# kennychenfs/KataCoffee

Measured on AMD Instinct MI355X. Metric: self-play training rows/sec + MCTS playouts/sec, 5x5 Coffee b6c96 @600 visits, higher is better.
Workload: dtype fp16

## Files before the change

katacoffee_amd/csrc/nn.hip:

```cpp
#include <hip/hip_runtime.h>
#include <hip/hip_ext.h>

#include <algorithm>
#include <cmath>
#include <cstring>
#include <functional>
#include <mutex>
#include <vector>

#include "detmath.h"
#include "engine.h"
#include "kc_board.h"
#include "lds_dma.h"

namespace kc {

typedef _Float16 h16x8 __attribute__((ext_vector_type(8)));
typedef float f32x4 __attribute__((ext_vector_type(4)));

enum { NN_MODE_F16 = 0, NN_MODE_SPLIT3 = 1, NN_MODE_F8C = 2 };
constexpr int F8C_SHIFT = 11;
constexpr float F8C_MAX = 448.0f;
#ifndef KC_F8C_VGPR
#define KC_F8C_VGPR 96
// ... 27 lines not shown
  const float f = std::frexp(m, &e);
  const int s = e - 9 + (f > 0.875f ? 1 : 0);
  return s < -100 ? -100 : (s > 100 ? 100 : s);
}

template <int X_, int Y_, int C_, int NB_ = NN_BOARDS_PER_WG, int MODE_ = 0, bool BL_ = false>
struct NNGeo {
  static constexpr int X = X_, Y = Y_, C = C_, A = X_ * Y_;
  static constexpr int NB = NB_;
  static constexpr int NW = 8, NT = NW * 64;
  static constexpr int MODE = MODE_;
  static constexpr bool SPLIT = MODE_ != NN_MODE_F16;
  static constexpr int PLANES = SPLIT ? 2 : 1;
  static constexpr bool BL = BL_;
  static constexpr bool F8W = MODE_ == NN_MODE_F8C && KC_F8C_CVTW;
  static constexpr bool F8X = MODE_ == NN_MODE_F8C && KC_F8C_CVTX;
  static constexpr int RING = BL ? ((F8W || F8X) ? 3 : 2) : ((NB_ == NN_SMALL_NB && !SPLIT) ? 4 : 3);
  static constexpr bool PAIRS = RING == 4;
  static constexpr int ROWS = NB * A;
  static constexpr int RT = (ROWS + 15) / 16;
  static constexpr int RGROUPS = NW / 2;
  static constexpr int MAXT = (RT + RGROUPS - 1) / RGROUPS;
  static constexpr int MROWS = RGROUPS * MAXT * 16;
  static constexpr int PX = X + 2, PY = Y + 2, PA = PX * PY;
  static constexpr int ZROW = MROWS;
  static constexpr int PROWS = BL ? MROWS + 1 : NB * PA;
  static constexpr int ASTR = C + 16;
  static constexpr int ROWB = ASTR * 2;
  static constexpr int NCT = C / 32;
  static constexpr int NCT_ALL = C / 16;
  static constexpr int P = 4 * A;
  static constexpr int PLANE_BYTES = (PROWS * ROWB + 15) / 16 * 16;
  static constexpr int ROWB2 = F8X ? ROWB / 2 : ROWB;
  static constexpr int PLANE2_BYTES = SPLIT ? (PROWS * ROWB2 + 15) / 16 * 16 : 0;
  static constexpr int ACT_BYTES = PLANE_BYTES + PLANE2_BYTES;
  static constexpr int SCR = 36;
  static constexpr int OFF_SCR = MROWS * SCR * 4 > 96 * 64 * 4 ? MROWS * SCR * 4 : 96 * 64 * 4;
  static constexpr int OFF_POOL = ACT_BYTES;
  static constexpr int OFF_BIAS = OFF_POOL + 2 * NB * 96 * 4;
  static constexpr int WBUF = (C / 32) * NCT_ALL * 64;
  static constexpr int WBUF2 = !SPLIT ? 0 : (F8W ? WBUF / 2 : WBUF);
  static constexpr int WSLOT = (BL && !SPLIT) ? 3 * WBUF : WBUF + WBUF2;
  static constexpr int SLOT_PIECES = WSLOT / 64;
  static constexpr int tapPieces(int ncb) { return ncb * NCT_ALL * (!SPLIT ? 2 : (F8W ? 3 : 4)) / 2; }
  static constexpr int chunkTaps(int ncb, int ntaps) {
    return SLOT_PIECES / tapPieces(ncb) < 1 ? 1 : (SLOT_PIECES / tapPieces(ncb) < ntaps ? SLOT_PIECES / tapPieces(ncb) : ntaps);
  }
  static constexpr int chunks(int ncb, int ntaps) { return (ntaps + chunkTaps(ncb, ntaps) - 1) / chunkTaps(ncb, ntaps); }
  static constexpr int firstChunkPieces(int ncb, int ntaps) { return chunkTaps(ncb, ntaps) * tapPieces(ncb); }
  static constexpr int NTAB = 2 * MROWS + ROWS;
  static constexpr int OFF_TAB = OFF_BIAS + NB * 64 * 4;
  static constexpr int RING_VH = (32 + 64) * 96 * 4;
  static constexpr int NPRM = NN_PRM;
  static constexpr int OFF_PRM = (OFF_TAB + NTAB * 2 + 15) / 16 * 16;
  static constexpr int OFF_W = OFF_PRM + 2 * NPRM * 4;
  static constexpr int LDS = OFF_W + RING * WSLOT * 16;
  static constexpr bool SCR_IN_RING = BL && !SPLIT;
  static constexpr int SCR_OFF = SCR_IN_RING ? OFF_W + WSLOT * 16 : OFF_SCR;
  static_assert(C % 32 == 0, "C must be a multiple of 32");
  static_assert(SCR_IN_RING ? (MROWS * SCR * 4 <= WSLOT * 16 && RING == 2 && RING_VH + NB * 64 * 4 <= WSLOT * 16)
                            : OFF_SCR + MROWS * SCR * 4 <= ACT_BYTES,
                "f32 branch scratch must fit in act (or in ring slot 1)");
  static_assert(96 * 64 * 4 <= OFF_SCR, "gpool linear weights must fit below scr");
  static_assert(RING * WSLOT * 16 >= RING_VH + NB * 64 * 4, "head linear weights and vh must fit in the ring");
  static_assert((PLANES - 1) * PLANE_BYTES + (BL ? 0 : 2 * PA * ROWB) + 2 * 64 < 65536,
                "A-read offsets must fit the ds_read immediate");
  static_assert(!BL || C == 96, "borderless instances: b6c96");
  static_assert(LDS <= 163840, "LDS budget");
};

#ifdef KC_NN_PROFILE
__device__ unsigned long long g_nnPhase[4][64];
#define NN_PHASE(i)                                  \
  do {                                               \
    if(blockIdx.x < 4 && threadIdx.x == 0) {         \
      g_nnPhase[blockIdx.x][(i)] = clock64();        \
      if((i) == 0 || (i) == 42)                      \
        g_nnPhase[blockIdx.x][(i) == 0 ? 62 : 63] =  \
            __builtin_amdgcn_s_memrealtime();        \
    }                                                \
  } while(0)
#else
#define NN_PHASE(i) \
  do {              \
  } while(0)
#endif

KC_D uint16_t f16bits(float f) { return __builtin_bit_cast(uint16_t, (_Float16)f); }

template <class G>
KC_D int padCell(int b, int p) {
  const int y = p / G::X, x = p - y * G::X;
  return b * G::PA + (y + 1) * G::PX + x + 1;
}

template <class G>
KC_D void aBases(int (&ab)[G::MAXT], const uint16_t* rowPa, int tstart, int lane) {
#pragma unroll
  for(int t = 0; t < G::MAXT; t++) {
    const int r = (tstart + t) * 16 + (lane & 15);
    ab[t] = ((int)rowPa[r] - G::PX - 1) * G::ROWB + 16 * (lane >> 4);
  }
}

template <int NW>
KC_D void stageTapDma(const h16x8* __restrict__ src, uint32_t slotAddr, int ch, int wave, int lane, int rot = 0) {
  for(int c = (wave + NW - rot % NW) % NW; c < ch; c += NW)
    glds16s(src + c * 64, (uint32_t)lane * 16u, slotAddr + c * 1024);
}

template <class G, int NTAPS, int NCB, int PAR = 0, int DBG = 0, bool ENTRY = true>
KC_D void convTiles(const uint16_t* __restrict__ act, const h16x8* __restrict__ w, h16x8* __restrict__ wl,
                    f32x4 (&acc)[G::MAXT][G::NCT], const int (&ab)[G::MAXT], int cg, int lane, int tid,
                    const h16x8* __restrict__ wNext, int chNext, int nextTaps, int g0 = 0) {
  constexpr int CHP = NCB * G::NCT_ALL;
  constexpr int CH = CHP * G::PLANES;
  constexpr int UNITS = CH * 64;
  constexpr int STEPS = NTAPS * NCB;
  const int wave = __builtin_amdgcn_readfirstlane(tid >> 6);
  const uint32_t ring = ldsAddr(wl);
  auto slotOf = [&](int tap) { return G::PAIRS ? (g0 + tap) & 3 : tap % 3; };
  if(ENTRY && !(DBG & 256)) {
    waitVm<0>();
    __syncthreads();
  }
  const char* actB = reinterpret_cast<const char*>(act);
  const h16x8* wlane = wl + (cg * G::NCT) * 64 + lane;
  h16x8 af[2][G::MAXT], bf[2][G::NCT];
  h16x8 afl[G::SPLIT ? 2 : 1][G::MAXT], bfl[G::SPLIT ? 2 : 1][G::NCT];
  auto loadStep = [&](int st, int buf) {
    const int tap = st / NCB, cb = st - tap * NCB;
    const int tb = NTAPS == 9 ? tap : 4;
    const int aoff = ((tb / 3) * G::PX + tb % 3) * G::ROWB + cb * 64;
    const h16x8* wb = wlane + slotOf(tap) * G::WSLOT + cb * G::NCT_ALL * 64;
#pragma unroll
    for(int ct = 0; ct < G::NCT; ct++) {
      bf[buf][ct] = wb[ct * 64];
// ... 248 lines not shown
    }
    if constexpr(F8C) {
      convertStep(st & 1);
      if((st & 1) && !(DBG & 4))
        f8pair();
    }
    if(chunkEnd && chunk + 1 < NCH && (DBG & 2) && !(DBG & 1))
      request(chunk + R);
    constexpr bool LATE = (F8C && KC_F8C_LATE) || (G::MODE == NN_MODE_SPLIT3 && G::BL && KC_ACC_LATE);
    if(!LATE && st + 1 < STEPS && !(DBG & 16)) {
      if(cb == NCB - 1)
        tapAddr(tap + 1);
      loadStep(st + 1, (st + 1) & 1);
    }
    __builtin_amdgcn_sched_barrier(0);
    const int b = st & 1;
#pragma unroll
    for(int t = 0; t < G::MAXT; t++)
#pragma unroll
      for(int ct = 0; ct < G::NCT; ct++)
        acc[t][ct] = __builtin_amdgcn_mfma_f32_16x16x32_f16(bf[b][ct], af[b][t], acc[t][ct], 0, 0, 0);
    if constexpr(G::MODE == NN_MODE_SPLIT3) {
#pragma unroll
      for(int t = 0; t < G::MAXT; t++)
#pragma unroll
        for(int ct = 0; ct < G::NCT; ct++)
          acc[t][ct] = __builtin_amdgcn_mfma_f32_16x16x32_f16(bfl[b][ct], af[b][t], acc[t][ct], 0, 0, 0);
#pragma unroll
      for(int t = 0; t < G::MAXT; t++)
#pragma unroll
        for(int ct = 0; ct < G::NCT; ct++)
          acc[t][ct] = __builtin_amdgcn_mfma_f32_16x16x32_f16(bf[b][ct], afl[b][t], acc[t][ct], 0, 0, 0);
    }
    if(LATE && st + 1 < STEPS) {
      __builtin_amdgcn_sched_barrier(0);
      if(cb == NCB - 1)
        tapAddr(tap + 1);
      loadStep(st + 1, (st + 1) & 1);
    }
    if constexpr(F8C) {
      if(st == STEPS - 1 && !(st & 1) && !(DBG & 4)) {
#pragma unroll
        for(int t = 0; t < G::MAXT; t++)
          aq[t].hi = i32x4{0, 0, 0, 0};
        f8pair();
      }
    }
    __builtin_amdgcn_sched_barrier(0);
  }
}

typedef _Float16 f16x4 __attribute__((ext_vector_type(4)));

template <int NT>
KC_D void stage96(float* __restrict__ dst, const float* __restrict__ src, int rows, int tid) {
  const int n4 = rows * 24;
  for(int q = tid; q < n4; q += NT)
    reinterpret_cast<float4*>(dst)[q] = reinterpret_cast<const float4*>(src)[q];
}

template <class G>
KC_D f32x4* trunkBase(float* trunk, int wave, int lane) {
  return reinterpret_cast<f32x4*>(trunk) + ((size_t)blockIdx.x * G::NW + wave) * (G::MAXT * G::NCT * 64) + lane;
}
template <class G>
constexpr bool regTrunk() {
  return G::MAXT * G::NCT <= 6 && !(G::MODE == NN_MODE_F8C && KC_F8C_PARK);
}
template <class G>
KC_D void storeTrunk(float* trunk, f32x4 (&reg)[G::MAXT][G::NCT], const f32x4 (&a)[G::MAXT][G::NCT], int wave,
                     int lane) {
  if(regTrunk<G>()) {
#pragma unroll
    for(int t = 0; t < G::MAXT; t++)
#pragma unroll
      for(int ct = 0; ct < G::NCT; ct++)
        reg[t][ct] = a[t][ct];
    return;
  }
  f32x4* p = trunkBase<G>(trunk, wave, lane);
#pragma unroll
  for(int t = 0; t < G::MAXT; t++)
#pragma unroll
    for(int ct = 0; ct < G::NCT; ct++)
      p[(t * G::NCT + ct) * 64] = a[t][ct];
}
template <class G>
KC_D void loadTrunk(f32x4 (&a)[G::MAXT][G::NCT], const f32x4 (&reg)[G::MAXT][G::NCT], float* trunk, int wave,
                    int lane) {
  if(regTrunk<G>()) {
#pragma unroll
    for(int t = 0; t < G::MAXT; t++)
#pragma unroll
      for(int ct = 0; ct < G::NCT; ct++)
        a[t][ct] = reg[t][ct];
    return;
  }
  const f32x4* p = trunkBase<G>(trunk, wave, lane);
#pragma unroll
  for(int t = 0; t < G::MAXT; t++)
#pragma unroll
    for(int ct = 0; ct < G::NCT; ct++)
      a[t][ct] = p[(t * G::NCT + ct) * 64];
}

template <class G>
KC_D void zeroAcc(f32x4 (&a)[G::MAXT][G::NCT]) {
#pragma unroll
  for(int t = 0; t < G::MAXT; t++)
#pragma unroll
    for(int ct = 0; ct < G::NCT; ct++)
      a[t][ct] = f32x4{0.0f, 0.0f, 0.0f, 0.0f};
}
// ... 59 lines not shown
                      int nb = 0) {
  float4 sc[G::NCT], bi[G::NCT];
#pragma unroll
  for(int ct = 0; ct < G::NCT; ct++) {
    const int ch = chOf<G>(cg, ct, lane);
    sc[ct] = *reinterpret_cast<const float4*>(s + ch);
    bi[ct] = *reinterpret_cast<const float4*>(bb + ch);
  }
  float m[G::MAXT];
#pragma unroll
  for(int t = 0; t < G::MAXT; t++) {
    m[t] = 0.0f;
    const int row = (tstart + t) * 16 + (lane & 15);
    if(row >= G::ROWS)
      continue;
#pragma unroll
    for(int ct = 0; ct < G::NCT; ct++) {
      const float y0 = fmaxf((float)v[t][ct][0] * sc[ct].x + bi[ct].x, 0.0f);
      const float y1 = fmaxf((float)v[t][ct][1] * sc[ct].y + bi[ct].y, 0.0f);
      const float y2 = fmaxf((float)v[t][ct][2] * sc[ct].z + bi[ct].z, 0.0f);
      const float y3 = fmaxf((float)v[t][ct][3] * sc[ct].w + bi[ct].w, 0.0f);
      storeAct4<G>(act, (int)rowPa[row], chOf<G>(cg, ct, lane), y0, y1, y2, y3);
      if constexpr(G::MODE == NN_MODE_F8C)
        m[t] = fmaxf(m[t], fmaxf(fmaxf(y0, y1), fmaxf(y2, y3)));
    }
  }
  flagHot<G>(hot, base, nb, tstart, lane, m);
}

template <class G>
KC_D void zeroBorders(uint16_t* act, int tid) {
  constexpr int CH = G::ASTR / 8;
  constexpr int NBORD = G::PA - G::A;
  for(int idx = tid; idx < G::NB * NBORD * CH; idx += G::NT) {
    const int q = idx / CH, c = idx - q * CH;
    const int b = q / NBORD, k = q - b * NBORD;
    int cell;
    if(k < G::PX)
      cell = k;
    else if(k < 2 * G::PX)
      cell = (G::PY - 1) * G::PX + (k - G::PX);
    else {
      const int m = k - 2 * G::PX;
      cell = (1 + (m >> 1)) * G::PX + ((m & 1) ? G::PX - 1 : 0);
    }
#pragma unroll
    for(int pl = 0; pl < G::PLANES; pl++)
      reinterpret_cast<uint4*>(act + pl * (G::PLANE_BYTES / 2) + (b * G::PA + cell) * G::ASTR)[c] = uint4{0u, 0u, 0u, 0u};
  }
}

template <class G>
KC_D void poolBoards(const float* scr, const float* vsrc, float* poolP, float* poolV, float sqOff, int tid) {
  for(int idx = tid; idx < G::NB * 64; idx += G::NT) {
    const int pr = idx >> 1, half = idx & 1;
    const int b = pr >> 5, c = pr & 31;
    const int p0 = half ? (G::A + 1) / 2 : 0, p1 = half ? G::A : (G::A + 1) / 2;
    float s = 0.0f, m = 0.0f, sv = 0.0f;
#pragma unroll 4
    for(int p = p0; p < p1; p++) {
      const int o = (b * G::A + p) * G::SCR + c;
      const float v = scr[o];
      s += v;
      m = v > m ? v : m;
      if(vsrc)
        sv += vsrc[o];
    }
    s = s + asF(partner<5>(bitsF(s)));
    m = fmaxf(m, asF(partner<5>(bitsF(m))));
    if(vsrc)
      sv = sv + asF(partner<5>(bitsF(sv)));
    if(half == 0) {
      const float mean = s / (float)G::A;
      poolP[b * 96 + c] = mean;
      poolP[b * 96 + 32 + c] = mean * (sqOff / 10.0f);
      poolP[b * 96 + 64 + c] = m;
      if(vsrc) {
        const float meanv = sv / (float)G::A;
        poolV[b * 96 + c] = meanv;
        poolV[b * 96 + 32 + c] = meanv * (sqOff / 10.0f);
        poolV[b * 96 + 64 + c] = meanv * ((sqOff * sqOff) / 100.0f - 0.1f);
      }
    }
  }
}

template <class G>
KC_D void linear96(const float* wT, int O, const float* in, float* out, int ostr, const float* bias, bool relu,
                   int tid) {
  const int quads = O >> 2;
  auto dot = [&](int q, int ks, int b) {
    float4 s = float4{0.0f, 0.0f, 0.0f, 0.0f};
    const float* xi = in + b * 96 + ks * 24;
    const float* wi = wT + (ks * 24) * O + 4 * q;
#pragma unroll 4
    for(int i = 0; i < 24; i++) {
      const float4 w4 = *reinterpret_cast<const float4*>(wi + i * O);
      const float xv = xi[i];
      s.x += w4.x * xv;
      s.y += w4.y * xv;
      s.z += w4.z * xv;
      s.w += w4.w * xv;
    }
    return s;
  };
  auto emit = [&](const float4& s, int q, int b) {
    float r[4] = {s.x, s.y, s.z, s.w};
#pragma unroll
    for(int j = 0; j < 4; j++) {
      float v = bias ? bias[4 * q + j] + r[j] : r[j];
      out[b * ostr + 4 * q + j] = relu ? fmaxf(v, 0.0f) : v;
    }
  };
  auto add2 = [](float& x, int lvl) {
    int a0, a1;
    if(lvl == 0)
      swapPair<0>(bitsF(x), a0, a1);
    else
      swapPair<1>(bitsF(x), a0, a1);
    x = asF(a0) + asF(a1);
  };
  if(quads == 16 || quads == 8) {
    const int per = 4 * quads;
    for(int idx = tid; idx < G::NB * per; idx += G::NT) {
      const int q = idx & (quads - 1), ks = (idx / quads) & 3, b = idx / per;
      float4 s = dot(q, ks, b);
      if(quads == 16) {
        add2(s.x, 1);
        add2(s.y, 1);
        add2(s.z, 1);
        add2(s.w, 1);
        add2(s.x, 0);
        add2(s.y, 0);
        add2(s.z, 0);
        add2(s.w, 0);
      } else {
        s.x += asF(partner<2>(bitsF(s.x)));
        s.y += asF(partner<2>(bitsF(s.y)));
        s.z += asF(partner<2>(bitsF(s.z)));
        s.w += asF(partner<2>(bitsF(s.w)));
        add2(s.x, 1);
        add2(s.y, 1);
        add2(s.z, 1);
        add2(s.w, 1);
      }
      if(ks == 0)
        emit(s, q, b);
    }
    return;
  }
  for(int idx = tid; idx < G::NB * quads * 4; idx += G::NT) {
    const int ks = idx & 3, q = (idx >> 2) % quads, b = (idx >> 2) / quads;
    float4 s = dot(q, ks, b);
    s.x += asF(partner<5>(bitsF(s.x)));
    s.y += asF(partner<5>(bitsF(s.y)));
    s.z += asF(partner<5>(bitsF(s.z)));
    s.w += asF(partner<5>(bitsF(s.w)));
    s.x += asF(partner<4>(bitsF(s.x)));
    s.y += asF(partner<4>(bitsF(s.y)));
    s.z += asF(partner<4>(bitsF(s.z)));
    s.w += asF(partner<4>(bitsF(s.w)));
    if(ks == 0)
      emit(s, q, b);
  }
}

KC_D float loadParam(const NNLayout* __restrict__ L, const float* __restrict__ WF, int k, int tid) {
  return tid < NN_PRM ? WF[L->prmSlabs + k * NN_PRM + tid] : 0.0f;
}
static int paramSlabSource(const NNLayout& L, int k, int tid) {
  const int f = tid < 384 ? tid / 96 : (tid < 416 ? 4 : 5), i = tid < 384 ? tid - 96 * f : (tid - 384) & 31;
  if(k < L.nblocks) {
    if(f == 0) return L.bn1s[k] + i;
    if(f == 1) return L.bn1b[k] + i;
    if(f == 2) return L.bn2s[k] + i;
    if(f == 3) return L.bn2b[k] + i;
    if(tid < NN_PRM && L.kinds[k] == 1) return (f == 4 ? L.bngs[k] : L.bngb[k]) + i;
    return -1;
  }
  if(tid >= 288) return -1;
  if(tid < 96) return L.tips + tid;
  if(tid < 192) return L.tipb + tid - 96;
  if(tid < 224) return L.pBiasG + tid - 192;
  if(tid < 256) return L.vBias1 + tid - 224;
  return L.pBias2 + tid - 256;
}

#ifndef KC_NN_KERNEL
#define KC_NN_KERNEL kNNForward
#define KC_NN_KERNEL_ATTR
#endif
template <int X, int Y, int C, int NB, int MODE, bool BL>
__global__ void __launch_bounds__(512, 2) KC_NN_KERNEL_ATTR
    KC_NN_KERNEL(const NNLayout* __restrict__ L, const h16x8* __restrict__ WB, const float* __restrict__ WF,
               const uint16_t* __restrict__ tabs, int n, const int* __restrict__ countDev,
               const int* __restrict__ rowIdx, int inWords, float winLen, const uint64_t* __restrict__ in,
               float* __restrict__ out, float* __restrict__ trunk, int* __restrict__ hot) {
  using G = NNGeo<X, Y, C, NB, MODE, BL>;
  extern __shared__ __attribute__((aligned(16))) char smem[];
  NN_PHASE(0);
  const int count = countDev ? min(*countDev, n) : n;
  const int base = blockIdx.x * G::NB;
  if(base >= count)
    return;
  const int nb = min(G::NB, count - base);
  uint32_t hotMask = ~0u;
  if(G::MODE == NN_MODE_SPLIT3 && hot) {
    hotMask = 0;
    for(int b = 0; b < nb; b++)
      hotMask |= __hip_atomic_load(hot + base + b, __ATOMIC_RELAXED, __HIP_MEMORY_SCOPE_AGENT) ? 1u << b : 0u;
    if(!hotMask)
      return;
  }
  const int tid = threadIdx.x, wave = tid >> 6, lane = tid & 63;
  const int rg = wave >> 1, cg = wave & 1;
  const int tstart = rg * G::MAXT;
  uint16_t* act = reinterpret_cast<uint16_t*>(smem);
  float* actF = reinterpret_cast<float*>(smem);
  float* scr = reinterpret_cast<float*>(smem + G::SCR_OFF);
  float* poolP = reinterpret_cast<float*>(smem + G::OFF_POOL);
  float* poolV = poolP + G::NB * 96;
  float* biasS = reinterpret_cast<float*>(smem + G::OFF_BIAS);
  float* vh = reinterpret_cast<float*>(smem + G::OFF_W + G::RING_VH);
  uint16_t* rowPa = reinterpret_cast<uint16_t*>(smem + G::OFF_TAB);
  uint16_t* rowBP = rowPa + G::MROWS;
  float* prm = reinterpret_cast<float*>(smem + G::OFF_PRM);
  h16x8* wl = reinterpret_cast<h16x8*>(smem + G::OFF_W);
  const float sqOff = sqrtf((float)G::A) - 14.0f;

  {
    constexpr int CH0 = G::tapPieces(1);
    const uint32_t ring = ldsAddr(wl);
    if constexpr(G::BL) {
      constexpr int SC = G::firstChunkPieces(1, 9);
#pragma unroll
      for(int j = 0; j + 1 < G::RING && j < G::chunks(1, 9); j++)
        stageChunk<G::NW>(WB + L->wInit + (size_t)j * SC * 64, ring + j * G::WSLOT * 16, SC, wave, lane);
    } else {
#pragma unroll
      for(int tap = 0; tap < 2; tap++)
        stageTapDma<G::NW>(WB + L->wInit + (size_t)tap * CH0 * 64, ring + tap * G::WSLOT * 16, CH0, wave, lane);
    }
  }
  constexpr int NPK = (G::NPRM + G::NT - 1) / G::NT;
  float pre[NPK];
#pragma unroll
  for(int j = 0; j < NPK; j++)
    pre[j] = loadParam(L, WF, 0, tid + j * G::NT);
  for(int i = tid; i < G::NTAB; i += G::NT)
    rowPa[i] = tabs[i];
  for(int idx = tid; idx < G::ACT_BYTES / 16; idx += G::NT)
    reinterpret_cast<uint4*>(smem)[idx] = uint4{0u, 0u, 0u, 0u};
  __syncthreads();
  {
    static_assert(G::NB <= G::NW, "one wave per board");
    constexpr int NBITS = G::A * NUM_SPATIAL, NWD = (NBITS + 63) / 64;
    const int b = __builtin_amdgcn_readfirstlane(wave);
    if(b < nb) {
      const int src = rowIdx ? rowIdx[base + b] : base + b;
      uint64_t words[NWD];
#pragma unroll
      for(int k = 0; k < NWD; k++)
        words[k] = in[(size_t)src * inWords + k];
#pragma unroll
      for(int k = 0; k < NWD; k++) {
        const int i = k * 64 + lane;
        if(i < NBITS && ((words[k] >> lane) & 1ULL)) {
          const int c = i / G::A, p = i - c * G::A;
          const int row = G::BL ? b * G::A + p : padCell<G>(b, p);
          act[row * G::ASTR + c] = (uint16_t)0x3c00;
          if constexpr(G::MODE == NN_MODE_F8C && !G::F8X)
            reinterpret_cast<uint8_t*>(act)[G::PLANE_BYTES + row * G::ROWB + (c >> 3) * 16 + (c & 7)] = 0x38;
        }
      }
    }
  }
  waitVm<0>();
  __syncthreads();

  NN_PHASE(1);
  int ab[G::MAXT];
  int rb[G::MAXT];
  uint32_t vm[G::MAXT];
  if constexpr(G::BL)
    aRowsBL<G>(rb, vm, tstart, lane);
  else
    aBases<G>(ab, rowPa, tstart, lane);
  f32x4 acc[G::MAXT][G::NCT];
  f32x4 park[G::MAXT][G::NCT];
  zeroAcc<G>(acc);
  if constexpr(G::BL)
    convTilesB<G, 9, 1, 0>(act, WB + L->wInit, wl, acc, rb, vm, cg, lane, tid,
                           L->nblocks > 0 ? WB + L->wConv1[0] : WB + L->wHead,
                           L->nblocks > 0 ? G::firstChunkPieces(G::C / 32, 9) : G::firstChunkPieces(G::C / 32, 1),
                           L->nblocks > 0 ? G::chunks(G::C / 32, 9) : 1, L->sInit);
  else
    convTiles<G, 9, 1, 0, 0, false>(act, WB + L->wInit, wl, acc, ab, cg, lane, tid,
                                    L->nblocks > 0 ? WB + L->wConv1[0] : WB + L->wHead, 3 * G::NCT_ALL * G::PLANES,
                                    L->nblocks > 0 ? 9 : 1, 0);
  {
#pragma unroll
    for(int ct = 0; ct < G::NCT; ct++) {
      const float4 g4 = *reinterpret_cast<const float4*>(WF + L->globInit + chOf<G>(cg, ct, lane));
#pragma unroll
      for(int t = 0; t < G::MAXT; t++) {
        acc[t][ct][0] += g4.x * winLen;
        acc[t][ct][1] += g4.y * winLen;
        acc[t][ct][2] += g4.z * winLen;
        acc[t][ct][3] += g4.w * winLen;
      }
    }
  }
// ... 13 lines not shown
    barrierKeepDma();
    NN_PHASE(3 + 4 * blk);
    const float* P = prm + (blk & 1) * G::NPRM;
    storeBnRelu<G>(act, rowPa, acc, P, P + 96, tstart, cg, lane, hot, base, nb);
    waitVm<0>();
    __syncthreads();
    zeroAcc<G>(acc);
#pragma unroll
    for(int j = 0; j < NPK; j++)
      pre[j] = loadParam(L, WF, blk + 1, tid + j * G::NT);
    NN_PHASE(4 + 4 * blk);
    if constexpr(G::BL)
      convTilesB<G, 9, G::C / 32, G::RING == 2 ? 1 : 0>(act, WB + L->wConv1[blk], wl, acc, rb, vm, cg, lane, tid,
                                                       WB + L->wConv2[blk],
                                                       L->kinds[blk] == 0 ? G::firstChunkPieces(3, 9)
                                                                          : G::firstChunkPieces(2, 9),
                                                       L->kinds[blk] == 0 ? G::chunks(3, 9) : G::chunks(2, 9),
                                                       L->sConv1[blk]);
    else
      convTiles<G, 9, G::C / 32, 1, 0, false>(act, WB + L->wConv1[blk], wl, acc, ab, cg, lane, tid,
                                              WB + L->wConv2[blk],
                                              (L->kinds[blk] == 0 ? 3 : 2) * G::NCT_ALL * G::PLANES, 9, 9 + 18 * blk);
#pragma unroll
    for(int j = 0; j < NPK; j++)
      if(tid + j * G::NT < G::NPRM)
        prm[((blk + 1) & 1) * G::NPRM + tid + j * G::NT] = pre[j];
    __syncthreads();
    NN_PHASE(5 + 4 * blk);
    const bool lastBlk = blk + 1 == L->nblocks;
    const h16x8* nextW = lastBlk ? WB + L->wHead : WB + L->wConv1[lastBlk ? 0 : blk + 1];
    const int nextTaps = lastBlk ? 1 : 9;
    if(L->kinds[blk] == 0) {
      f32x4 tr[G::MAXT][G::NCT];
      loadTrunk<G>(tr, park, trunk, wave, lane);
      storeBnRelu<G>(act, rowPa, acc, P + 192, P + 288, tstart, cg, lane, hot, base, nb);
#pragma unroll
      for(int t = 0; t < G::MAXT; t++)
#pragma unroll
        for(int ct = 0; ct < G::NCT; ct++)
          acc[t][ct] = tr[t][ct];
      waitVm<0>();
      __syncthreads();
      NN_PHASE(6 + 4 * blk);
      if constexpr(G::BL)
        convTilesB<G, 9, G::C / 32, 0>(act, WB + L->wConv2[blk], wl, acc, rb, vm, cg, lane, tid, nextW,
                                       G::firstChunkPieces(G::C / 32, nextTaps), G::chunks(G::C / 32, nextTaps),
                                       L->sConv2[blk]);
      else
        convTiles<G, 9, G::C / 32, 0, 0, false>(act, WB + L->wConv2[blk], wl, acc, ab, cg, lane, tid, nextW,
                                                3 * G::NCT_ALL * G::PLANES, nextTaps, 18 + 18 * blk);
      if(!lastBlk)
        storeTrunk<G>(trunk, park, acc, wave, lane);
    } else {
      const float* gs = P + 384;
      const float* gbias = P + 416;
      constexpr int LW = (96 * 64 / 4 + G::NT - 1) / G::NT;
      float4 lw[LW];
      {
        const float4* src = reinterpret_cast<const float4*>(WF + L->linG[blk]);
#pragma unroll
        for(int k = 0; k < LW; k++) {
          const int q = tid + k * G::NT;
          lw[k] = q < Cr * 24 ? src[q] : float4{0.0f, 0.0f, 0.0f, 0.0f};
        }
      }
#pragma unroll
      for(int ct = 0; ct < G::NCT; ct++) {
        const int ch = chOf<G>(cg, ct, lane);
        if(cg * (G::C / 2) + ct * 16 < Cr)
          continue;
        const int gc = ch - Cr;
        const float4 sc = *reinterpret_cast<const float4*>(gs + gc);
        const float4 bi = *reinterpret_cast<const float4*>(gbias + gc);
#pragma unroll
        for(int t = 0; t < G::MAXT; t++) {
          const int row = (tstart + t) * 16 + (lane & 15);
          if(row >= G::ROWS)
            continue;
          *reinterpret_cast<float4*>(scr + (int)rowBP[row] * G::SCR + gc) =
              float4{fmaxf(acc[t][ct][0] * sc.x + bi.x, 0.0f), fmaxf(acc[t][ct][1] * sc.y + bi.y, 0.0f),
                     fmaxf(acc[t][ct][2] * sc.z + bi.z, 0.0f), fmaxf(acc[t][ct][3] * sc.w + bi.w, 0.0f)};
        }
      }
      __syncthreads();
      NN_PHASE(50);
      float* lgT = actF;
#pragma unroll
      for(int k = 0; k < LW; k++) {
        const int q = tid + k * G::NT;
        if(q < Cr * 24)
          reinterpret_cast<float4*>(lgT)[q] = lw[k];
      }
      poolBoards<G>(scr, nullptr, poolP, poolV, sqOff, tid);
      __syncthreads();
      NN_PHASE(51);
      linear96<G>(lgT, Cr, poolP, biasS, Cr, nullptr, false, tid);
      __syncthreads();
      f32x4 tr[G::MAXT][G::NCT];
      loadTrunk<G>(tr, park, trunk, wave, lane);
      if constexpr(G::BL)
        zeroRowBL<G>(act, tid);
      else
        zeroBorders<G>(act, tid);
      NN_PHASE(52);
      {
        const float* s2 = P + 192;
        const float* b2 = P + 288;
        float m[G::MAXT] = {};
#pragma unroll
        for(int ct = 0; ct < G::NCT; ct++) {
          if(cg * (G::C / 2) + ct * 16 >= Cr)
            continue;
          const int ch = chOf<G>(cg, ct, lane);
          const float4 sc = *reinterpret_cast<const float4*>(s2 + ch);
          const float4 bi = *reinterpret_cast<const float4*>(b2 + ch);
#pragma unroll
          for(int t = 0; t < G::MAXT; t++) {
            const int row = (tstart + t) * 16 + (lane & 15);
            if(row >= G::ROWS)
              continue;
            const float4 gb = *reinterpret_cast<const float4*>(biasS + ((int)rowBP[row] / G::A) * Cr + ch);
            const float y0 = fmaxf((acc[t][ct][0] + gb.x) * sc.x + bi.x, 0.0f);
            const float y1 = fmaxf((acc[t][ct][1] + gb.y) * sc.y + bi.y, 0.0f);
            const float y2 = fmaxf((acc[t][ct][2] + gb.z) * sc.z + bi.z, 0.0f);
            const float y3 = fmaxf((acc[t][ct][3] + gb.w) * sc.w + bi.w, 0.0f);
            storeAct4<G>(act, (int)rowPa[row], ch, y0, y1, y2, y3);
            if constexpr(G::MODE == NN_MODE_F8C)
              m[t] = fmaxf(m[t], fmaxf(fmaxf(y0, y1), fmaxf(y2, y3)));
          }
        }
        flagHot<G>(hot, base, nb, tstart, lane, m);
      }
#pragma unroll
      for(int t = 0; t < G::MAXT; t++)
#pragma unroll
        for(int ct = 0; ct < G::NCT; ct++)
          acc[t][ct] = tr[t][ct];
      waitVm<0>();
      __syncthreads();
      NN_PHASE(6 + 4 * blk);
      if constexpr(G::BL)
        convTilesB<G, 9, (G::C - 32) / 32, 0>(act, WB + L->wConv2[blk], wl, acc, rb, vm, cg, lane, tid, nextW,
                                              G::firstChunkPieces(G::C / 32, nextTaps),
                                              G::chunks(G::C / 32, nextTaps), L->sConv2[blk]);
      else
        convTiles<G, 9, (G::C - 32) / 32, 0, 0, false>(act, WB + L->wConv2[blk], wl, acc, ab, cg, lane, tid, nextW,
                                                       3 * G::NCT_ALL * G::PLANES, nextTaps, 18 + 18 * blk);
      if(!lastBlk)
        storeTrunk<G>(trunk, park, acc, wave, lane);
    }
  }
  __syncthreads();
  NN_PHASE(40);
  const float* PT = prm + (L->nblocks & 1) * G::NPRM;
  storeBnRelu<G>(act, rowPa, acc, PT, PT + 96, tstart, cg, lane, hot, base, nb);
  waitVm<0>();
  __syncthreads();
  zeroAcc<G>(acc);
  if constexpr(G::BL)
    convTilesB<G, 1, G::C / 32, G::RING == 2 ? 1 : 0>(act, WB + L->wHead, wl, acc, rb, vm, cg, lane, tid, nullptr, 0,
                                                      0, L->sHead);
  else
    convTiles<G, 1, G::C / 32, 1, 0, false>(act, WB + L->wHead, wl, acc, ab, cg, lane, tid, nullptr, 0, 0,
                                            9 + 18 * L->nblocks);
  __syncthreads();
  NN_PHASE(41);
  {
    const float* pbg = PT + 192;
    const float* vb1 = PT + 224;
#pragma unroll
    for(int ct = 0; ct < G::NCT; ct++) {
      const int c0 = cg * (G::C / 2) + ct * 16;
      if(c0 < 32)
        continue;
      const bool isG = c0 < 64;
      const int hc = chOf<G>(cg, ct, lane) - (isG ? 32 : 64);
      const float4 bi = *reinterpret_cast<const float4*>((isG ? pbg : vb1) + hc);
      float* dst = isG ? scr : actF;
#pragma unroll
      for(int t = 0; t < G::MAXT; t++) {
        const int row = (tstart + t) * 16 + (lane & 15);
        if(row >= G::ROWS)
          continue;
        *reinterpret_cast<float4*>(dst + (int)rowBP[row] * G::SCR + hc) =
            float4{fmaxf(acc[t][ct][0] + bi.x, 0.0f), fmaxf(acc[t][ct][1] + bi.y, 0.0f),
                   fmaxf(acc[t][ct][2] + bi.z, 0.0f), fmaxf(acc[t][ct][3] + bi.w, 0.0f)};
      }
    }
  }
  __syncthreads();
  NN_PHASE(53);
  float* plgT = reinterpret_cast<float*>(wl);
  float* l2T = plgT + 32 * 96;
  float* w3 = prm + ((L->nblocks + 1) & 1) * G::NPRM;
  static_assert(4 * 64 + 4 <= G::NPRM, "value weights fit a parameter slab");
  stage96<G::NT>(plgT, WF + L->pLinG, 32, tid);
  stage96<G::NT>(l2T, WF + L->vLin2, L->v2, tid);
  {
    const int v2 = L->v2;
    for(int i = tid; i < 4 * v2 + 4; i += G::NT) {
      float w;
      if(i < 2 * v2)
        w = WF[L->vLin3 + i];
      else if(i < 4 * v2)
        w = WF[L->vLinM + i - 2 * v2];
      else
        w = i - 4 * v2 < 2 ? WF[L->vB3 + i - 4 * v2] : WF[L->vBM + i - 4 * v2 - 2];
      w3[i] = w;
    }
  }
  poolBoards<G>(scr, actF, poolP, poolV, sqOff, tid);
  __syncthreads();
  NN_PHASE(54);
  linear96<G>(plgT, 32, poolP, biasS, 32, nullptr, false, tid);
  linear96<G>(l2T, L->v2, poolV, vh, 64, WF + L->vB2, true, tid);
  __syncthreads();
  {
    static_assert(G::NB * 4 * 16 <= G::NT, "one 16-lane group per (board, output)");
    const int k = tid & 15, o = (tid >> 4) & 3, b = tid >> 6;
    const int v2 = L->v2;
    const int bv = b < G::NB ? b : 0;
    float s = 0.0f;
    for(int i = k; i < v2; i += 16)
      s += w3[o * v2 + i] * vh[bv * 64 + i];
    s += asF(partner<2>(bitsF(s)));
    s += asF(partner<3>(bitsF(s)));
    s += asF(partner<4>(bitsF(s)));
    s += asF(partner<5>(bitsF(s)));
    if(k == 0 && b < nb && ((hotMask >> b) & 1u)) {
      const int dst = rowIdx ? rowIdx[base + b] : base + b;
      out[(size_t)dst * (G::P + 4) + G::P + o] = s + w3[4 * v2 + o];
    }
  }
  NN_PHASE(42);
  if(cg == 0) {
    const float* pb2 = PT + 256;
    const float* w2 = WF + L->pConv2;
    const int c0 = chOf<G>(0, 0, lane), c1 = chOf<G>(0, 1, lane);
#pragma unroll
    for(int t = 0; t < G::MAXT; t++) {
      const int row = (tstart + t) * 16 + (lane & 15);
      const int bp = row < G::ROWS ? (int)rowBP[row] : 0;
      const int brd = bp / G::A;
      float pv[8];
#pragma unroll
      for(int j = 0; j < 4; j++) {
        pv[j] = fmaxf(acc[t][0][j] + biasS[brd * 32 + c0 + j] + pb2[c0 + j], 0.0f);
        pv[4 + j] = fmaxf(acc[t][1][j] + biasS[brd * 32 + c1 + j] + pb2[c1 + j], 0.0f);
      }
      float part[4];
#pragma unroll
      for(int d = 0; d < 4; d++) {
        float s = 0.0f;
#pragma unroll
        for(int j = 0; j < 4; j++)
          s += pv[j] * w2[d * 32 + c0 + j] + pv[4 + j] * w2[d * 32 + c1 + j];
        {
          int a0, a1;
          swapPair<1>(bitsF(s), a0, a1);
          s = asF(a0) + asF(a1);
          swapPair<0>(bitsF(s), a0, a1);
          s = asF(a0) + asF(a1);
        }
        part[d] = s;
      }
      if((lane >> 4) == 0 && row < G::ROWS && brd < nb && ((hotMask >> brd) & 1u)) {
        const int pp = bp - brd * G::A;
        float* o = out + (size_t)(rowIdx ? rowIdx[base + brd] : base + brd) * (G::P + 4);
#pragma unroll
        for(int d = 0; d < 4; d++)
          o[d * G::A + pp] = part[d];
      }
    }
  }
  if(G::MODE == NN_MODE_SPLIT3 && hot && tid < nb)
    hot[base + tid] = 0;
}

#ifndef KC_NN_KERNEL_ONLY
#if KC_F8C_VGPR
template <int X, int Y, int C, int NB, int MODE, bool BL>
__global__ void kNNForwardCap(const NNLayout* __restrict__ L, const h16x8* __restrict__ WB,
                              const float* __restrict__ WF, const uint16_t* __restrict__ tabs, int n,
                              const int* __restrict__ countDev, const int* __restrict__ rowIdx, int inWords,
                              float winLen, const uint64_t* __restrict__ in, float* __restrict__ out,
                              float* __restrict__ trunk, int* __restrict__ hot);
#endif
template <class G>
constexpr auto nnKernel() {
#if KC_F8C_VGPR
  if constexpr(G::MODE == NN_MODE_F8C || (G::MODE == NN_MODE_F16 && G::BL) ||
               (KC_ACC_CAP && G::MODE == NN_MODE_SPLIT3 && G::BL))
    return kNNForwardCap<G::X, G::Y, G::C, G::NB, G::MODE, G::BL>;
  else
#endif
    return kNNForward<G::X, G::Y, G::C, G::NB, G::MODE, G::BL>;
}


static uint16_t f2h(float f) {
  uint32_t u;
  memcpy(&u, &f, 4);
  const uint32_t sign = (u >> 16) & 0x8000u, a = u & 0x7fffffffu;
  if(a >= 0x7f800000u)
    return (uint16_t)(sign | 0x7c00u | (a > 0x7f800000u ? 0x200u : 0u));
  if(a < 0x38800000u) {
    float m;
    memcpy(&m, &a, 4);
    return (uint16_t)(sign | (uint32_t)nearbyintf(m * 16777216.0f));
  }
  uint32_t r = a + 0xfffu + ((a >> 13) & 1u);
  if(r >= 0x47800000u)
    return (uint16_t)(sign | 0x7c00u);
  return (uint16_t)(sign | (((r >> 23) - 112u) << 10) | ((r >> 13) & 0x3ffu));
}

static float h2f(uint16_t h) {
  const uint32_t sign = (uint32_t)(h & 0x8000u) << 16, e = (h >> 10) & 0x1fu, m = h & 0x3ffu;
  float f;
  if(e == 0) {
    f = ldexpf((float)m, -24);
  } else if(e == 31) {
    const uint32_t u = 0x7f800000u | (m << 13);
    memcpy(&f, &u, 4);
  } else {
    const uint32_t u = ((e + 112u) << 23) | (m << 13);
    memcpy(&f, &u, 4);
  }
  uint32_t u;
// ... 269 lines not shown
    return ci < cfg_.cin ? m.convInit[((size_t)co * cfg_.cin + ci) * 9 + tap] : 0.0f;
  }, wmode, &L.sInit);
  L.globInit = f32(m.globInit);
  for(int i = 0; i < L.nblocks; i++) {
    const ModelBlock& b = m.blocks[i];
    L.kinds[i] = b.kind;
    L.bn1s[i] = f32(b.bn1s);
    L.bn1b[i] = f32(b.bn1b);
    L.wConv1[i] = bfOff();
    if(b.kind == 0) {
      packConv(wb, 9, C, C, [&](int co, int ci, int tap) { return b.conv1[((size_t)co * C + ci) * 9 + tap]; }, wmode,
               &L.sConv1[i]);
      L.bn2s[i] = f32(b.bn2s);
      L.bn2b[i] = f32(b.bn2b);
      L.wConv2[i] = bfOff();
      packConv(wb, 9, C, C, [&](int co, int ci, int tap) { return b.conv2[((size_t)co * C + ci) * 9 + tap]; }, wmode,
               &L.sConv2[i]);
    } else {
      packConv(wb, 9, C, C, [&](int co, int ci, int tap) {
        return co < Cr ? b.conv1[((size_t)co * C + ci) * 9 + tap] : b.conv1g[((size_t)(co - Cr) * C + ci) * 9 + tap];
      }, wmode, &L.sConv1[i]);
      L.bngs[i] = f32(b.bngs);
      L.bngb[i] = f32(b.bngb);
      L.linG[i] = f32T(b.linG, Cr);
      L.bn2s[i] = f32(b.bn2s);
      L.bn2b[i] = f32(b.bn2b);
      L.wConv2[i] = bfOff();
      packConv(wb, 9, Cr, C, [&](int co, int ci, int tap) { return b.conv2[((size_t)co * Cr + ci) * 9 + tap]; },
               wmode, &L.sConv2[i]);
    }
  }
  L.tips = f32(m.tips);
  L.tipb = f32(m.tipb);
  L.wHead = bfOff();
  packConv(wb, 1, C, C, [&](int co, int ci, int) {
    if(co < 32)
      return m.pConv1[(size_t)co * C + ci];
    if(co < 64)
      return m.pConvG[(size_t)(co - 32) * C + ci];
    return m.vConv1[(size_t)(co - 64) * C + ci];
  }, wmode, &L.sHead);
  L.pBiasG = f32(m.pBiasG);
  L.pLinG = f32T(m.pLinG, 32);
  L.pBias2 = f32(m.pBias2);
  L.pConv2 = f32(m.pConv2);
  L.vBias1 = f32(m.vBias1);
  L.vLin2 = f32T(m.vLin2, cfg_.v2);
  L.vB2 = f32(m.vB2);
  L.vLin3 = f32(m.vLin3);
  L.vB3 = f32(m.vB3);
  L.vLinM = f32(m.vLinM);
  L.vBM = f32(m.vBM);
  {
    std::vector<float> slabs((size_t)(L.nblocks + 1) * NN_PRM);
    for(int k = 0; k <= L.nblocks; k++)
      for(int t = 0; t < NN_PRM; t++) {
        const int src = paramSlabSource(L, k, t);
        slabs[(size_t)k * NN_PRM + t] = src >= 0 ? wf[src] : 0.0f;
      }
    L.prmSlabs = f32(slabs);
  }
  KC_HIP(hipMalloc(&wHalf_, wb.size() * 2));
  KC_HIP(hipMemcpy(wHalf_, wb.data(), wb.size() * 2, hipMemcpyHostToDevice));
  KC_HIP(hipMalloc(&wF32_, wf.size() * 4));
  KC_HIP(hipMemcpy(wF32_, wf.data(), wf.size() * 4, hipMemcpyHostToDevice));
  KC_HIP(hipMalloc(&layoutDev_, sizeof(NNLayout)));
  KC_HIP(hipMemcpy(layoutDev_, &L, sizeof(NNLayout), hipMemcpyHostToDevice));
  using G8 = NNGeo<5, 5, 96, 8, 0>;
  using G4 = NNGeo<5, 5, 96, NN_SMALL_NB, 0>;
  using GS = NNGeo<5, 5, 96, 2, NN_MODE_SPLIT3>;
  using GB = NNGeo<5, 5, 96, NN_SMALL_NB, NN_MODE_SPLIT3, true>;
  using GC = NNGeo<5, 5, 96, NN_SMALL_NB, NN_MODE_F8C, true>;
  const std::vector<uint16_t> tab8 = rowTables<G8>(), tab4 = rowTables<G4>(), tabS = rowTables<GS>(),
                              tabB = rowTables<GB>();
  KC_HIP(hipMalloc(&tabDevB_, tabB.size() * 2));
  KC_HIP(hipMemcpy(tabDevB_, tabB.data(), tabB.size() * 2, hipMemcpyHostToDevice));
  KC_HIP(hipMalloc(&tabDev_, tab8.size() * 2));
  KC_HIP(hipMemcpy(tabDev_, tab8.data(), tab8.size() * 2, hipMemcpyHostToDevice));
  KC_HIP(hipMalloc(&tabDevSm_, tab4.size() * 2));
  KC_HIP(hipMemcpy(tabDevSm_, tab4.data(), tab4.size() * 2, hipMemcpyHostToDevice));
  KC_HIP(hipMalloc(&tabDevS_, tabS.size() * 2));
  KC_HIP(hipMemcpy(tabDevS_, tabS.data(), tabS.size() * 2, hipMemcpyHostToDevice));

  KC_HIP(hipFuncSetAttribute((const void*)kNNForward<5, 5, 96, 8, 0, false>, hipFuncAttributeMaxDynamicSharedMemorySize,
                             G8::LDS));
  KC_HIP(hipFuncSetAttribute((const void*)kNNForward<5, 5, 96, NN_SMALL_NB, 0, false>, hipFuncAttributeMaxDynamicSharedMemorySize,
                             G4::LDS));
  KC_HIP(hipFuncSetAttribute((const void*)kNNForward<5, 5, 96, 2, NN_MODE_SPLIT3, false>,
                             hipFuncAttributeMaxDynamicSharedMemorySize, GS::LDS));
  KC_HIP(hipFuncSetAttribute((const void*)kNNForward<5, 5, 96, NN_SMALL_NB, NN_MODE_SPLIT3, true>,
                             hipFuncAttributeMaxDynamicSharedMemorySize, GB::LDS));
  KC_HIP(hipFuncSetAttribute((const void*)nnKernel<GC>(), hipFuncAttributeMaxDynamicSharedMemorySize, GC::LDS));
  using GF = NNGeo<5, 5, 96, NN_SMALL_NB, 0, true>;
  KC_HIP(hipFuncSetAttribute((const void*)nnKernel<GF>(), hipFuncAttributeMaxDynamicSharedMemorySize, GF::LDS));
#ifdef KC_AB_HOOKS
  const char* small = getenv("KATACOFFEE_NN_SMALL");
  small_ = small ? atoi(small) : 0;
#endif
  int dev = 0;
  KC_HIP(hipGetDevice(&dev));
  KC_HIP(hipDeviceGetAttribute(&cus_, hipDeviceAttributeMultiprocessorCount, dev));
}

NNEngine::~NNEngine() { release(); }

void NNEngine::release() {
  for(void* p : {(void*)trunk_, wHalf_, (void*)wF32_, (void*)layoutDev_, (void*)tabDev_, (void*)tabDevSm_,
                 (void*)tabDevS_, (void*)tabDevB_, (void*)hot_})
// ... 157 lines not shown
```

Before: 29120.

## Prefetch head weights into registers during the final conv and fuse head linears

Head weights (policy gpool linear, value linear 2, value-3/mean weights and biases, policy conv2) are now prefetched into registers during the last trunk conv and written to LDS after it, so their global-load latency overlaps compute instead of stalling the head. An extra parameter slab is packed on the host for these values. The two head linear layers become one fused loop, pooling loads are unrolled into registers, and destination row indices are cached in LDS. Extra profiling phase markers are also added. The cost is more register pressure during the trunk's final conv and some extra LDS.

```diff
diff --git a/katacoffee_amd/csrc/nn.hip b/katacoffee_amd/csrc/nn.hip
--- a/katacoffee_amd/csrc/nn.hip
+++ b/katacoffee_amd/csrc/nn.hip
@@ -103,7 +103,8 @@
   static constexpr int OFF_TAB = OFF_BIAS + NB * 64 * 4;
   static constexpr int RING_VH = (32 + 64) * 96 * 4;
   static constexpr int NPRM = NN_PRM;
-  static constexpr int OFF_PRM = (OFF_TAB + NTAB * 2 + 15) / 16 * 16;
+  static constexpr int OFF_DST = (OFF_TAB + NTAB * 2 + 3) / 4 * 4;
+  static constexpr int OFF_PRM = (OFF_DST + NB * 4 + 15) / 16 * 16;
   static constexpr int OFF_W = OFF_PRM + 2 * NPRM * 4;
   static constexpr int LDS = OFF_W + RING * WSLOT * 16;
   static constexpr bool SCR_IN_RING = BL && !SPLIT;
@@ -126,14 +127,30 @@
   do {                                               \
     if(blockIdx.x < 4 && threadIdx.x == 0) {         \
       g_nnPhase[blockIdx.x][(i)] = clock64();        \
-      if((i) == 0 || (i) == 42)                      \
-        g_nnPhase[blockIdx.x][(i) == 0 ? 62 : 63] =  \
+      if((i) == 42)                                  \
+        g_nnPhase[blockIdx.x][63] =                  \
             __builtin_amdgcn_s_memrealtime();        \
     }                                                \
+  } while(0)
+#define NN_PHASE_ENTRY()                       \
+  const unsigned long long nnT0 = clock64(),   \
+                           nnR0 = __builtin_amdgcn_s_memrealtime()
+#define NN_PHASE_ENTRY_COMMIT()                \
+  do {                                         \
+    if(blockIdx.x < 4 && threadIdx.x == 0) {   \
+      g_nnPhase[blockIdx.x][0] = nnT0;         \
+      g_nnPhase[blockIdx.x][62] = nnR0;        \
+    }                                          \
   } while(0)
 #else
 #define NN_PHASE(i) \
   do {              \
+  } while(0)
+#define NN_PHASE_ENTRY() \
+  do {                   \
+  } while(0)
+#define NN_PHASE_ENTRY_COMMIT() \
+  do {                          \
   } while(0)
 #endif
 
@@ -488,13 +505,6 @@
 
 typedef _Float16 f16x4 __attribute__((ext_vector_type(4)));
 
-template <int NT>
-KC_D void stage96(float* __restrict__ dst, const float* __restrict__ src, int rows, int tid) {
-  const int n4 = rows * 24;
-  for(int q = tid; q < n4; q += NT)
-    reinterpret_cast<float4*>(dst)[q] = reinterpret_cast<const float4*>(src)[q];
-}
-
 template <class G>
 KC_D f32x4* trunkBase(float* trunk, int wave, int lane) {
   return reinterpret_cast<f32x4*>(trunk) + ((size_t)blockIdx.x * G::NW + wave) * (G::MAXT * G::NCT * 64) + lane;
@@ -660,19 +670,28 @@
 
 template <class G>
 KC_D void poolBoards(const float* scr, const float* vsrc, float* poolP, float* poolV, float sqOff, int tid) {
+  constexpr int H = (G::A + 1) / 2;
   for(int idx = tid; idx < G::NB * 64; idx += G::NT) {
     const int pr = idx >> 1, half = idx & 1;
     const int b = pr >> 5, c = pr & 31;
-    const int p0 = half ? (G::A + 1) / 2 : 0, p1 = half ? G::A : (G::A + 1) / 2;
+    const int cnt = half ? G::A - H : H;
+    const int o0 = (b * G::A + (half ? H : 0)) * G::SCR + c;
+    float v[H], vv[H];
+#pragma unroll
+    for(int i = 0; i < H; i++) {
+      v[i] = i < cnt ? scr[o0 + i * G::SCR] : 0.0f;
+      if(vsrc)
+        vv[i] = i < cnt ? vsrc[o0 + i * G::SCR] : 0.0f;
+    }
     float s = 0.0f, m = 0.0f, sv = 0.0f;
-#pragma unroll 4
-    for(int p = p0; p < p1; p++) {
-      const int o = (b * G::A + p) * G::SCR + c;
-      const float v = scr[o];
-      s += v;
-      m = v > m ? v : m;
-      if(vsrc)
-        sv += vsrc[o];
+#pragma unroll
+    for(int i = 0; i < H; i++) {
+      if(i < cnt) {
+        s += v[i];
+        m = v[i] > m ? v[i] : m;
+        if(vsrc)
+          sv += vv[i];
+      }
     }
     s = s + asF(partner<5>(bitsF(s)));
     m = fmaxf(m, asF(partner<5>(bitsF(m))));
@@ -773,6 +792,57 @@
   }
 }
 
+template <int O>
+KC_D void linear96Item(const float* wT, const float* in, float* out, const float* bias, bool relu, int idx) {
+  static_assert(O == 64 || O == 32, "a board's items are a wave or an aligned half of one");
+  constexpr int quads = O >> 2;
+  const int q = idx & (quads - 1), ks = (idx / quads) & 3, b = idx / (4 * quads);
+  float4 s = float4{0.0f, 0.0f, 0.0f, 0.0f};
+  const float* xi = in + b * 96 + ks * 24;
+  const float* wi = wT + (ks * 24) * O + 4 * q;
+#pragma unroll 4
+  for(int i = 0; i < 24; i++) {
+    const float4 w4 = *reinterpret_cast<const float4*>(wi + i * O);
+    const float xv = xi[i];
+    s.x += w4.x * xv;
+    s.y += w4.y * xv;
+    s.z += w4.z * xv;
+    s.w += w4.w * xv;
+  }
+  float r[4] = {s.x, s.y, s.z, s.w};
+#pragma unroll
+  for(int j = 0; j < 4; j++) {
+    int a0, a1;
+    if(O == 64) {
+      swapPair<1>(bitsF(r[j]), a0, a1);
+      r[j] = asF(a0) + asF(a1);
+      swapPair<0>(bitsF(r[j]), a0, a1);
+      r[j] = asF(a0) + asF(a1);
+    } else {
+      r[j] += asF(partner<2>(bitsF(r[j])));
+      swapPair<1>(bitsF(r[j]), a0, a1);
+      r[j] = asF(a0) + asF(a1);
+    }
+  }
+  if(ks == 0) {
+#pragma unroll
+    for(int j = 0; j < 4; j++) {
+      const float v = bias ? bias[4 * q + j] + r[j] : r[j];
+      out[b * O + 4 * q + j] = relu ? fmaxf(v, 0.0f) : v;
+    }
+  }
+}
+template <class G>
+KC_D void headLinears(const float* plgT, const float* poolP, float* biasS, const float* l2T, const float* poolV,
+                      float* vh, const float* vB2, int tid) {
+  for(int idx = tid; idx < G::NB * 96; idx += G::NT) {
+    if(idx < G::NB * 64)
+      linear96Item<64>(l2T, poolV, vh, vB2, true, idx);
+    else
+      linear96Item<32>(plgT, poolP, biasS, nullptr, false, idx - G::NB * 64);
+  }
+}
+
 KC_D float loadParam(const NNLayout* __restrict__ L, const float* __restrict__ WF, int k, int tid) {
   return tid < NN_PRM ? WF[L->prmSlabs + k * NN_PRM + tid] : 0.0f;
 }
@@ -786,7 +856,16 @@
     if(tid < NN_PRM && L.kinds[k] == 1) return (f == 4 ? L.bngs[k] : L.bngb[k]) + i;
     return -1;
   }
-  if(tid >= 288) return -1;
+  if(k == L.nblocks + 1) {
+    const int v2 = L.v2;
+    if(tid < 2 * v2) return L.vLin3 + tid;
+    if(tid < 4 * v2) return L.vLinM + tid - 2 * v2;
+    if(tid < 4 * v2 + 2) return L.vB3 + tid - 4 * v2;
+    if(tid < 4 * v2 + 4) return L.vBM + tid - 4 * v2 - 2;
+    if(tid < 5 * v2 + 4) return L.vB2 + tid - 4 * v2 - 4;
+    return -1;
+  }
+  if(tid >= 288) return tid < 288 + 4 * L.p1 && tid < 416 ? L.pConv2 + tid - 288 : -1;
   if(tid < 96) return L.tips + tid;
   if(tid < 192) return L.tipb + tid - 96;
   if(tid < 224) return L.pBiasG + tid - 192;
@@ -806,7 +885,7 @@
                float* __restrict__ out, float* __restrict__ trunk, int* __restrict__ hot) {
   using G = NNGeo<X, Y, C, NB, MODE, BL>;
   extern __shared__ __attribute__((aligned(16))) char smem[];
-  NN_PHASE(0);
+  NN_PHASE_ENTRY();
   const int count = countDev ? min(*countDev, n) : n;
   const int base = blockIdx.x * G::NB;
   if(base >= count)
@@ -820,6 +899,7 @@
     if(!hotMask)
       return;
   }
+  NN_PHASE_ENTRY_COMMIT();
   const int tid = threadIdx.x, wave = tid >> 6, lane = tid & 63;
   const int rg = wave >> 1, cg = wave & 1;
   const int tstart = rg * G::MAXT;
@@ -834,6 +914,7 @@
   uint16_t* rowBP = rowPa + G::MROWS;
   float* prm = reinterpret_cast<float*>(smem + G::OFF_PRM);
   h16x8* wl = reinterpret_cast<h16x8*>(smem + G::OFF_W);
+  int* dstRow = reinterpret_cast<int*>(smem + G::OFF_DST);
   const float sqOff = sqrtf((float)G::A) - 14.0f;
 
   {
@@ -866,6 +947,8 @@
     const int b = __builtin_amdgcn_readfirstlane(wave);
     if(b < nb) {
       const int src = rowIdx ? rowIdx[base + b] : base + b;
+      if(lane == 0)
+        dstRow[b] = src;
       uint64_t words[NWD];
 #pragma unroll
       for(int k = 0; k < NWD; k++)
@@ -985,6 +1068,7 @@
       if(!lastBlk)
         storeTrunk<G>(trunk, park, acc, wave, lane);
     } else {
+      NN_PHASE(49);
       const float* gs = P + 384;
       const float* gbias = P + 416;
       constexpr int LW = (96 * 64 / 4 + G::NT - 1) / G::NT;
@@ -1071,6 +1155,7 @@
           acc[t][ct] = tr[t][ct];
       waitVm<0>();
       __syncthreads();
+      NN_PHASE(55);
       NN_PHASE(6 + 4 * blk);
       if constexpr(G::BL)
         convTilesB<G, 9, (G::C - 32) / 32, 0>(act, WB + L->wConv2[blk], wl, acc, rb, vm, cg, lane, tid, nextW,
@@ -1086,6 +1171,21 @@
   __syncthreads();
   NN_PHASE(40);
   const float* PT = prm + (L->nblocks & 1) * G::NPRM;
+#pragma unroll
+  for(int j = 0; j < NPK; j++)
+    pre[j] = loadParam(L, WF, L->nblocks + 1, tid + j * G::NT);
+  constexpr int HW = ((32 + 64) * 24 + G::NT - 1) / G::NT;
+  float4 hw[HW];
+  {
+    const float4* srcP = reinterpret_cast<const float4*>(WF + L->pLinG);
+    const float4* srcV = reinterpret_cast<const float4*>(WF + L->vLin2);
+    const int nV = L->v2 * 24;
+#pragma unroll
+    for(int k = 0; k < HW; k++) {
+      const int q = tid + k * G::NT;
+      hw[k] = q < 32 * 24 ? srcP[q] : (q - 32 * 24 < nV ? srcV[q - 32 * 24] : float4{0.0f, 0.0f, 0.0f, 0.0f});
+    }
+  }
   storeBnRelu<G>(act, rowPa, acc, PT, PT + 96, tstart, cg, lane, hot, base, nb);
   waitVm<0>();
   __syncthreads();
@@ -1098,6 +1198,20 @@
                                             9 + 18 * L->nblocks);
   __syncthreads();
   NN_PHASE(41);
+  float* plgT = reinterpret_cast<float*>(wl);
+  float* l2T = plgT + 32 * 96;
+  float* w3 = prm + ((L->nblocks + 1) & 1) * G::NPRM;
+  static_assert(4 * 64 + 4 + 64 <= G::NPRM, "value weights and biases fit a parameter slab");
+#pragma unroll
+  for(int j = 0; j < NPK; j++)
+    if(tid + j * G::NT < G::NPRM)
+      w3[tid + j * G::NT] = pre[j];
+#pragma unroll
+  for(int k = 0; k < HW; k++) {
+    const int q = tid + k * G::NT;
+    if(q < (32 + 64) * 24)
+      reinterpret_cast<float4*>(plgT)[q] = hw[k];
+  }
   {
     const float* pbg = PT + 192;
     const float* vb1 = PT + 224;
@@ -1123,31 +1237,20 @@
   }
   __syncthreads();
   NN_PHASE(53);
-  float* plgT = reinterpret_cast<float*>(wl);
-  float* l2T = plgT + 32 * 96;
-  float* w3 = prm + ((L->nblocks + 1) & 1) * G::NPRM;
-  static_assert(4 * 64 + 4 <= G::NPRM, "value weights fit a parameter slab");
-  stage96<G::NT>(plgT, WF + L->pLinG, 32, tid);
-  stage96<G::NT>(l2T, WF + L->vLin2, L->v2, tid);
-  {
-    const int v2 = L->v2;
-    for(int i = tid; i < 4 * v2 + 4; i += G::NT) {
-      float w;
-      if(i < 2 * v2)
-        w = WF[L->vLin3 + i];
-      else if(i < 4 * v2)
-        w = WF[L->vLinM + i - 2 * v2];
-      else
-        w = i - 4 * v2 < 2 ? WF[L->vB3 + i - 4 * v2] : WF[L->vBM + i - 4 * v2 - 2];
-      w3[i] = w;
-    }
-  }
+  NN_PHASE(56);
   poolBoards<G>(scr, actF, poolP, poolV, sqOff, tid);
   __syncthreads();
   NN_PHASE(54);
-  linear96<G>(plgT, 32, poolP, biasS, 32, nullptr, false, tid);
-  linear96<G>(l2T, L->v2, poolV, vh, 64, WF + L->vB2, true, tid);
+  if(L->v2 == 64) {
+    headLinears<G>(plgT, poolP, biasS, l2T, poolV, vh, w3 + 4 * 64 + 4, tid);
+    NN_PHASE(57);
+  } else {
+    linear96<G>(plgT, 32, poolP, biasS, 32, nullptr, false, tid);
+    NN_PHASE(57);
+    linear96<G>(l2T, L->v2, poolV, vh, 64, w3 + 4 * L->v2 + 4, true, tid);
+  }
   __syncthreads();
+  NN_PHASE(58);
   {
     static_assert(G::NB * 4 * 16 <= G::NT, "one 16-lane group per (board, output)");
     const int k = tid & 15, o = (tid >> 4) & 3, b = tid >> 6;
@@ -1161,14 +1264,13 @@
     s += asF(partner<4>(bitsF(s)));
     s += asF(partner<5>(bitsF(s)));
     if(k == 0 && b < nb && ((hotMask >> b) & 1u)) {
-      const int dst = rowIdx ? rowIdx[base + b] : base + b;
-      out[(size_t)dst * (G::P + 4) + G::P + o] = s + w3[4 * v2 + o];
+      out[(size_t)dstRow[b] * (G::P + 4) + G::P + o] = s + w3[4 * v2 + o];
     }
   }
   NN_PHASE(42);
   if(cg == 0) {
     const float* pb2 = PT + 256;
-    const float* w2 = WF + L->pConv2;
+    const float* w2 = PT + 288;
     const int c0 = chOf<G>(0, 0, lane), c1 = chOf<G>(0, 1, lane);
 #pragma unroll
     for(int t = 0; t < G::MAXT; t++) {
@@ -1199,7 +1301,7 @@
       }
       if((lane >> 4) == 0 && row < G::ROWS && brd < nb && ((hotMask >> brd) & 1u)) {
         const int pp = bp - brd * G::A;
-        float* o = out + (size_t)(rowIdx ? rowIdx[base + brd] : base + brd) * (G::P + 4);
+        float* o = out + (size_t)dstRow[brd] * (G::P + 4);
 #pragma unroll
         for(int d = 0; d < 4; d++)
           o[d * G::A + pp] = part[d];
@@ -1208,6 +1310,7 @@
   }
   if(G::MODE == NN_MODE_SPLIT3 && hot && tid < nb)
     hot[base + tid] = 0;
+  NN_PHASE(59);
 }
 
 #ifndef KC_NN_KERNEL_ONLY
@@ -1583,8 +1686,8 @@
   L.vLinM = f32(m.vLinM);
   L.vBM = f32(m.vBM);
   {
-    std::vector<float> slabs((size_t)(L.nblocks + 1) * NN_PRM);
-    for(int k = 0; k <= L.nblocks; k++)
+    std::vector<float> slabs((size_t)(L.nblocks + 2) * NN_PRM);
+    for(int k = 0; k <= L.nblocks + 1; k++)
       for(int t = 0; t < NN_PRM; t++) {
         const int src = paramSlabSource(L, k, t);
         slabs[(size_t)k * NN_PRM + t] = src >= 0 ? wf[src] : 0.0f;
```

Measured after the change: 29440, median of 6. +1.1%, better.
